# AI-ON/Few-Shot-Music-Generation

Measured on AMD Instinct MI355X. Metric: episodes/s (LSTM-baseline train step, synthetic vocab=10k seq_len=128 5-way/5-shot h=512), higher is better.
Workload: dtype f32 (bf16x3-split products, fp32 accumulate)

## Files before the change

few-shot-music-generation_amd/csrc/api_debug.hip:

```cpp
#include "fsmg_model.h"

using namespace fsmg;
using namespace fsmg_host;


extern "C" {

int fsmg_debug_clock_begin(fsmg_handle h, int32_t microseconds) {
    if (!h || microseconds <= 0 || microseconds > 1000000) return FSMG_ERR_INVALID;
    BEGIN_CALL(h, true);
    if (!h->probe) HIPCK(h, hipStreamCreateWithFlags(&h->probe, hipStreamNonBlocking));
    if (!h->d_probe) HIPCK(h, hipMalloc((void**)&h->d_probe, 64));
    HIPCK(h, hipMemsetAsync(h->d_probe, 0, 64, h->probe));
    HIPCK(h, launch_clock_probe(h->probe, (long long)microseconds * 100, h->d_probe));
    return FSMG_OK;
}
int fsmg_debug_clock_end(fsmg_handle h, float* ghz) {
    if (!h || !ghz) return FSMG_ERR_INVALID;
    if (!h->probe || !h->d_probe) return fail(h, FSMG_ERR_STATE, "fsmg_debug_clock_end without fsmg_debug_clock_begin");
    BEGIN_CALL(h, true);
    unsigned long long v[2] = {0, 0};
    HIPCK(h, hipStreamSynchronize(h->probe));
    HIPCK(h, hipMemcpy(v, h->d_probe, sizeof(v), hipMemcpyDeviceToHost));
    *ghz = v[1] ? (float)((double)v[0] / (double)v[1] * 0.1) : 0.0f;
    return FSMG_OK;
}

int fsmg_debug_dims(fsmg_handle h, int32_t dims[5]) {
    if (!h || !dims) return FSMG_ERR_INVALID;
    dims[0] = h->Ep; dims[1] = h->Hp; dims[2] = h->V1p; dims[3] = h->lastB; dims[4] = h->T;
    return FSMG_OK;
}

int fsmg_debug_read(fsmg_handle h, const char* what, float* host, int64_t count) {
    if (!h || !what || !host || count <= 0) return FSMG_ERR_INVALID;
    BEGIN_CALL(h);
    const int64_t B = h->lastB, T = h->T, Hp = h->Hp, G4 = h->G4, rows = T * B;
    const float* src = nullptr; int64_t cap = 0;
    auto layer_of = [&](const char* prefix) -> int {
        const size_t n = std::strlen(prefix);
        if (std::strncmp(what, prefix, n) != 0) return -1;
        const int l = std::atoi(what + n);
        return (l >= 0 && l < h->L && std::strlen(what) > n) ? l : -1;
    };
    int l;
    if (!std::strcmp(what, "aux_tries")) { host[0] = (float)h->aux_tries; return FSMG_OK; }
    if (!std::strcmp(what, "fused_softmax")) { host[0] = h->fused_softmax ? 1.0f : 0.0f; if (count > 1) host[1] = h->fs_call ? 1.0f : 0.0f; return FSMG_OK; }
    if (!std::strcmp(what, "xcd_bx3")) { host[0] = h->xcd_bx3 ? 1.0f : 0.0f; return FSMG_OK; }
    if (!std::strcmp(what, "gemm_kinds")) {
        for (int64_t i = 0; i < count && i < 4; ++i) host[i] = (float)h->gemm_kinds[i];
        return FSMG_OK;
    }
    if (!std::strcmp(what, "xov_selfcheck")) {
        const float v[3] = {(float)h->xov_selfcheck_runs, (float)h->xov_passes, (float)h->xov_selfcheck_every};
        for (int64_t i = 0; i < count && i < 3; ++i) host[i] = v[i];
        return FSMG_OK;
    }
    if (!std::strcmp(what, "xcd_partitioned")) {
        host[0] = h->xov ? 1.0f : 0.0f;
        if (count > 1) { const int b = h->lastB > 0 ? h->lastB : 45, rpx = lstm_xcd16_packed_rows(b, h->Hp); host[1] = (h->xov && rpx > 0) ? (float)xov_first_free(b, h->Hp) : 8.0f; }
        if (count > 2) host[2] = h->xov_last ? 1.0f : 0.0f;
        return FSMG_OK;
    }
    if (!std::strcmp(what, "logits")) { src = h->logits; cap = rows * h->V1p; }
    else if (!std::strcmp(what, "dlogits")) { src = dlogits_buf(h); cap = rows * h->V1p; }
    else if (!std::strcmp(what, "lse")) { src = h->lse; cap = rows; }
    else if (!std::strcmp(what, "ce")) { src = h->ce; cap = rows; }
    else if (!std::strcmp(what, "dx")) { src = h->dXemb; cap = rows * h->Ep; }
    else if (!std::strcmp(what, "dh")) { src = h->dH; cap = rows * Hp; }
    else if (!std::strcmp(what, "gnorm")) { src = h->d_gnorm; cap = 1; }
    else if (!std::strcmp(what, "tail")) { src = h->G + h->n_flat; cap = FSMG_GRAD_TAIL; }
    else if ((l = layer_of("gates")) >= 0) { src = h->Z[l]; cap = rows * G4; }
    else if ((l = layer_of("h")) >= 0) { src = h->Hs[l]; cap = (T + 1) * B * Hp; }
    else if ((l = layer_of("c")) >= 0) { src = h->Cs[l]; cap = (T + 1) * B * Hp; }
    else return fail(h, FSMG_ERR_NAME, std::string("unknown debug buffer '") + what + "'");
    if (count > cap) return fail(h, FSMG_ERR_SIZE, "debug read larger than the buffer");
    HIPCK(h, hipStreamSynchronize(h->stream));
    HIPCK(h, hipMemcpy(host, src, sizeof(float) * count, hipMemcpyDeviceToHost));
    return FSMG_OK;
}

int fsmg_debug_step_profile(fsmg_handle h, int32_t which, uint64_t* stamps, int64_t cap, int32_t* n_blocks,
                            int32_t* n_waves) {
    if (!h || !stamps || !n_blocks || !n_waves || h->lastB <= 0 || h->T < 3) return FSMG_ERR_INVALID;
    BEGIN_CALL(h);
    { const int rc_cs = ensure_cs(h); if (rc_cs != FSMG_OK) return rc_cs; }
    const int B = h->lastB, Hp = h->Hp, G4 = h->G4, l = h->L - 1, t = h->T / 2;
    const int nb = which == 0 ? (G4 / 16) * ((B + 15) / 16) : (Hp / 16) * ((B + 15) / 16);
    const int nw = which == 0 ? 4 : 8;
    const int64_t n = (int64_t)nb * nw * 8;
    if (cap < n) return fail(h, FSMG_ERR_SIZE, "stamp buffer too small");
    unsigned long long* d = nullptr;
    HIPCK(h, hipMalloc((void**)&d, sizeof(unsigned long long) * n));
    HIPCK(h, hipMemsetAsync(d, 0, sizeof(unsigned long long) * n, h->stream));
    for (int rep = 0; rep < 3; ++rep) {
        if (which == 0) {
            LstmFwdArgs a{};
            const size_t Bp16 = (size_t)(B + 15) / 16 * 16;
            a.KhF = h->khf + (size_t)(2 * l) * Hp * G4; a.hF_prev = h->HF[l] + (size_t)t * Bp16 * Hp;
            a.hF_next = h->HF[l] + (size_t)(t + 1) * Bp16 * Hp; a.z = h->Z[l] + (size_t)t * B * G4;
            a.c_prev = h->Cs[l] + (size_t)t * B * Hp; a.c_next = h->Cs[l] + (size_t)(t + 1) * B * Hp;
            a.h_next = h->Hs[l] + (size_t)(t + 1) * B * Hp; a.B = B; a.Hp = Hp;
            HIPCK(h, launch_lstm_fwd_step(h->stream, a, d));
        } else {
            LstmBwdArgs a{};
            const size_t Bp16 = (size_t)(B + 15) / 16 * 16;
            a.KhF = h->khf + (size_t)(2 * l + 1) * Hp * G4; a.dzF_next = h->dzF + (size_t)((t + 1) & 1) * Bp16 * G4;
            a.dzF_cur = h->dzF + (size_t)(t & 1) * Bp16 * G4; a.gates = h->Z[l] + (size_t)t * B * G4;
            a.c_t = h->Cs[l] + (size_t)(t + 1) * B * Hp; a.c_prev = h->Cs[l] + (size_t)t * B * Hp; a.dc = h->dC;
            a.dh_top = h->dH + (size_t)t * B * Hp; a.B = B; a.Hp = Hp;
            HIPCK(h, launch_lstm_bwd_step(h->stream, a, d));
        }
    }
    HIPCK(h, hipStreamSynchronize(h->stream));
    HIPCK(h, hipMemcpy(stamps, d, sizeof(unsigned long long) * n, hipMemcpyDeviceToHost));
    hipFree(d);
    *n_blocks = nb; *n_waves = nw;
    return FSMG_OK;
}

int fsmg_timing_enable(fsmg_handle h, int32_t on) {
    if (!h) return FSMG_ERR_INVALID;
    BEGIN_CALL(h);
    drain_timers(h);
    h->timing = on != 0;
    return FSMG_OK;
}
int fsmg_timing_select(fsmg_handle h, const char* kernel_class) {
    if (!h) return FSMG_ERR_INVALID;
    BEGIN_CALL(h);
    drain_timers(h);
    h->timing_only = kernel_class ? kernel_class : "";
    return FSMG_OK;
}
int fsmg_timing_read(fsmg_handle h, const char* kernel_class, double* total_ms, int64_t* launches) {
    if (!h || !kernel_class) return FSMG_ERR_INVALID;
    BEGIN_CALL(h);
    drain_timers(h);
    auto it = h->timers.find(kernel_class);
    if (total_ms) *total_ms = it == h->timers.end() ? 0.0 : it->second.total_ms;
    if (launches) *launches = it == h->timers.end() ? 0 : it->second.launches;
    return FSMG_OK;
}
int fsmg_timing_reset(fsmg_handle h) {
    if (!h) return FSMG_ERR_INVALID;
    BEGIN_CALL(h);
    drain_timers(h);
    h->timers.clear();
    return FSMG_OK;
}

}
```

few-shot-music-generation_amd/csrc/elementwise.hip:

```cpp
#include <algorithm>
#include "fsmg_kernels.h"
#include <cstdlib>

namespace fsmg {
namespace {

__device__ __forceinline__ float wave_sum(float v) {
#pragma unroll
    for (int o = 32; o > 0; o >>= 1) v += __shfl_xor(v, o, 64);
    return v;
}
__device__ __forceinline__ double wave_sum_d(double v) {
#pragma unroll
    for (int o = 32; o > 0; o >>= 1) v += __shfl_xor(v, o, 64);
    return v;
}
__device__ __forceinline__ float wave_max(float v) {
#pragma unroll
    for (int o = 32; o > 0; o >>= 1) v = fmaxf(v, __shfl_xor(v, o, 64));
    return v;
}

__global__ __launch_bounds__(256) void k_fill32(uint32_t* __restrict__ p, uint32_t word, long long n) {
    const long long n4 = n >> 2;
    const uint4 w4 = make_uint4(word, word, word, word);
    for (long long i = (long long)blockIdx.x * 256 + threadIdx.x; i < n4; i += (long long)gridDim.x * 256)
        reinterpret_cast<uint4*>(p)[i] = w4;
    if (blockIdx.x == 0 && threadIdx.x < (n & 3)) p[(n4 << 2) + threadIdx.x] = word;
}

__global__ __launch_bounds__(256) void k_fill32_if(const int* __restrict__ cond, uint32_t* __restrict__ p, uint32_t word, long long n) {
    if (*cond == 0) return;
    const long long n4 = n >> 2;
    const uint4 w4 = make_uint4(word, word, word, word);
    for (long long i = (long long)blockIdx.x * 256 + threadIdx.x; i < n4; i += (long long)gridDim.x * 256)
        reinterpret_cast<uint4*>(p)[i] = w4;
    if (blockIdx.x == 0 && threadIdx.x < (n & 3)) p[(n4 << 2) + threadIdx.x] = word;
}

constexpr int SQ_CHUNK = 256 * 16;
__global__ __launch_bounds__(256) void k_multi_op(const MultiOps r) {
    const MultiOp& o = r.op[blockIdx.y];
    if (o.kind == MULTI_FILL) {
        if (o.cond != nullptr && *o.cond == 0) return;
        uint32_t* p = (uint32_t*)o.dst;
        const uint32_t word = o.word;
        const long long n = o.n, n4 = n >> 2;
        const uint4 w4 = make_uint4(word, word, word, word);
        for (long long i = (long long)blockIdx.x * 256 + threadIdx.x; i < n4; i += (long long)gridDim.x * 256)
            reinterpret_cast<uint4*>(p)[i] = w4;
        if (blockIdx.x == 0 && threadIdx.x < (n & 3)) p[(n4 << 2) + threadIdx.x] = word;
        return;
    }
    __shared__ double sh[4];
    if (o.kind == MULTI_MEAN) {
        if (blockIdx.x != 0) return;
        const int tid = threadIdx.x, lane = tid & 63, wave = tid >> 6;
        const float* x = (const float*)o.src;
        const int n = (int)o.n;
        double l = 0.0;
        for (int i0 = tid; i0 < n; i0 += 256 * 16) {
            float b[16];
#pragma unroll
            for (int k = 0; k < 16; ++k) b[k] = (i0 + 256 * k < n) ? x[i0 + 256 * k] : 0.0f;
#pragma unroll
            for (int k = 0; k < 16; ++k) if (i0 + 256 * k < n) l += (double)b[k];
        }
        l = wave_sum_d(l);
        if (lane == 0) sh[wave] = l;
        __syncthreads();
        if (tid == 0) *(float*)o.dst = (float)(((sh[0] + sh[1]) + (sh[2] + sh[3])) / ((double)n + 1e-12));
        return;
    }
    const int tid = threadIdx.x, lane = tid & 63, wave = tid >> 6;
    const float* sl = (const float*)o.src;
    float* out = (float*)o.dst;
    const long long n = o.n, nchunks = (n + SQ_CHUNK - 1) / SQ_CHUNK;
    const bool vec = (o.stride & 3) == 0 && (n & 3) == 0;
    if (o.sq == nullptr && vec) {
        const long long n4 = n >> 2;
        for (long long i = (long long)blockIdx.x * 256 + tid; i < n4; i += (long long)gridDim.x * 256) {
            float4 v = *reinterpret_cast<const float4*>(sl + 4 * i);
            int z = 1;
            for (; z + 3 < o.nslab; z += 4) {
                const float4 w0 = *reinterpret_cast<const float4*>(sl + z * o.stride + 4 * i);
                const float4 w1 = *reinterpret_cast<const float4*>(sl + (z + 1) * o.stride + 4 * i);
                const float4 w2 = *reinterpret_cast<const float4*>(sl + (z + 2) * o.stride + 4 * i);
                const float4 w3 = *reinterpret_cast<const float4*>(sl + (z + 3) * o.stride + 4 * i);
                v.x += w0.x; v.y += w0.y; v.z += w0.z; v.w += w0.w;
                v.x += w1.x; v.y += w1.y; v.z += w1.z; v.w += w1.w;
                v.x += w2.x; v.y += w2.y; v.z += w2.z; v.w += w2.w;
                v.x += w3.x; v.y += w3.y; v.z += w3.z; v.w += w3.w;
            }
            for (; z < o.nslab; ++z) {
                const float4 w = *reinterpret_cast<const float4*>(sl + z * o.stride + 4 * i);
                v.x += w.x; v.y += w.y; v.z += w.z; v.w += w.w;
            }
            if (o.row_scale != nullptr) {
                const float c = o.row_scale[(4 * i) / o.row_len];
                v.x *= c; v.y *= c; v.z *= c; v.w *= c;
            }
            *reinterpret_cast<float4*>(out + 4 * i) = v;
        }
        return;
    }
    for (long long c = blockIdx.x; c < nchunks; c += gridDim.x) {
        const long long base = c * SQ_CHUNK;
        double s = 0.0;
        if (vec && base + SQ_CHUNK <= n) {
            float4 v[4];
#pragma unroll
            for (int i = 0; i < 4; ++i) v[i] = *reinterpret_cast<const float4*>(sl + base + 4 * (tid + 256 * i));
            int z = 1;
            for (; z + 1 < o.nslab; z += 2) {
                float4 w0[4], w1[4];
#pragma unroll
                for (int i = 0; i < 4; ++i) {
                    w0[i] = *reinterpret_cast<const float4*>(sl + z * o.stride + base + 4 * (tid + 256 * i));
                    w1[i] = *reinterpret_cast<const float4*>(sl + (z + 1) * o.stride + base + 4 * (tid + 256 * i));
                }
#pragma unroll
                for (int i = 0; i < 4; ++i) {
                    v[i].x += w0[i].x; v[i].y += w0[i].y; v[i].z += w0[i].z; v[i].w += w0[i].w;
                    v[i].x += w1[i].x; v[i].y += w1[i].y; v[i].z += w1[i].z; v[i].w += w1[i].w;
                }
            }
            if (z < o.nslab) {
#pragma unroll
                for (int i = 0; i < 4; ++i) {
                    const float4 w = *reinterpret_cast<const float4*>(sl + z * o.stride + base + 4 * (tid + 256 * i));
                    v[i].x += w.x; v[i].y += w.y; v[i].z += w.z; v[i].w += w.w;
                }
            }
#pragma unroll
            for (int i = 0; i < 4; ++i) {
                *reinterpret_cast<float4*>(out + base + 4 * (tid + 256 * i)) = v[i];
                s += ((double)v[i].x * v[i].x + (double)v[i].y * v[i].y) + ((double)v[i].z * v[i].z + (double)v[i].w * v[i].w);
            }
        } else {
#pragma unroll
            for (int i = 0; i < 4; ++i) {
                const long long idx = base + 4 * (tid + 256 * i);
                float q[4] = {0.f, 0.f, 0.f, 0.f};
                int k = 0;
                for (long long j = idx; j < n && j < idx + 4; ++j, ++k) {
                    float v = sl[j];
                    for (int z = 1; z < o.nslab; ++z) v += sl[z * o.stride + j];
                    out[j] = v;
                    q[k] = v;
                }
                if (k == 4) s += ((double)q[0] * q[0] + (double)q[1] * q[1]) + ((double)q[2] * q[2] + (double)q[3] * q[3]);
                else for (int e = 0; e < k; ++e) s += (double)q[e] * q[e];
            }
        }
        if (o.sq != nullptr) {
            s = wave_sum_d(s);
            if (lane == 0) sh[wave] = s;
            __syncthreads();
            if (tid == 0) o.sq[c] = (sh[0] + sh[1]) + (sh[2] + sh[3]);
            __syncthreads();
        }
    }
}

__global__ void k_token_prep(const int* __restrict__ support, int n_support, const int* __restrict__ query,
                             int n_query, int T, int vocab, int start_word, int* __restrict__ X,
                             int* __restrict__ Y, int* __restrict__ err_flag, int* __restrict__ tok_first, int* __restrict__ tok_count) {
    __shared__ int s_key[512], s_cnt[512], s_min[512];
    const int B = n_support + n_query;
    const long long total = (long long)B * T;
    for (long long i0 = (long long)blockIdx.x * blockDim.x; i0 < total; i0 += (long long)gridDim.x * blockDim.x) {
        const long long i = i0 + threadIdx.x;
        const bool valid = i < total;
        const int b = valid ? (int)(i / T) : 0, t = valid ? (int)(i % T) : 0;
        int tok = 0;
        if (valid) {
            const int* row = (b < n_support) ? support + (long long)b * T : query + (long long)(b - n_support) * T;
            tok = row[t];
            if (tok < 0 || tok >= vocab) {
                atomicOr(err_flag, 1);
                tok = min(max(tok, 0), vocab - 1);
            }
            Y[(long long)t * B + b] = tok;
            if (t + 1 < T) X[(long long)(t + 1) * B + b] = tok;
            if (t == 0) X[b] = start_word;
        }
        if (tok_first != nullptr) {
            for (int j = threadIdx.x; j < 512; j += blockDim.x) { s_key[j] = -1; s_cnt[j] = 0; s_min[j] = 0x7FFFFFFF; }
            __syncthreads();
            if (valid && t + 1 < T) {
                const int pos = (int)((long long)(t + 1) * B + b);
                unsigned slot = ((unsigned)tok * 2654435761u) >> 23;
                bool placed = false;
#pragma unroll 1
                for (int probe = 0; probe < 8 && !placed; ++probe) {
                    const int prev = atomicCAS(&s_key[slot], -1, tok);
                    if (prev == -1 || prev == tok) { atomicAdd(&s_cnt[slot], 1); atomicMin(&s_min[slot], pos); placed = true; }
                    else slot = (slot + 1) & 511u;
                }
                if (!placed) { atomicMin(tok_first + tok, pos); atomicAdd(tok_count + tok, 1); }
            }
            __syncthreads();
            for (int j = threadIdx.x; j < 512; j += blockDim.x)
                if (s_key[j] >= 0) { atomicMin(tok_first + s_key[j], s_min[j]); atomicAdd(tok_count + s_key[j], s_cnt[j]); }
            __syncthreads();
            if (valid && t == 0) { atomicMin(tok_first + start_word, b); atomicAdd(tok_count + start_word, 1); }
        }
    }
}

__global__ void k_gather_rows(const int* __restrict__ table, const int* __restrict__ idx, int n_rows, int T, int n_songs,
                              int* __restrict__ out, int* __restrict__ err_flag) {
    const long long total = (long long)n_rows * T;
    for (long long i = (long long)blockIdx.x * blockDim.x + threadIdx.x; i < total; i += (long long)gridDim.x * blockDim.x) {
        const int r = (int)(i / T), t = (int)(i % T);
        int song = idx[r];
        if (song < 0 || song >= n_songs) { atomicOr(err_flag, 1); song = 0; }
        out[i] = table[(long long)song * T + t];
    }
}

__global__ __launch_bounds__(256) void k_ce_rows(const float* logits, int ld, int n_vocab,
                                                 const int* __restrict__ tgt, float* __restrict__ lse,
                                                 float* __restrict__ ce, float* dlogits, float inv_n) {
    __shared__ float sh[4];
    __shared__ float s_lse;
    const int r = blockIdx.x, tid = threadIdx.x, lane = tid & 63, wave = tid >> 6;
    const float* row = logits + (long long)r * ld;
    const int nv4 = n_vocab & ~3;
    float m = -INFINITY;
    for (int v = 4 * tid; v < nv4; v += 1024) {
        const float4 x = *reinterpret_cast<const float4*>(row + v);
        m = fmaxf(fmaxf(m, fmaxf(x.x, x.y)), fmaxf(x.z, x.w));
    }
    if (tid < n_vocab - nv4) m = fmaxf(m, row[nv4 + tid]);
    m = wave_max(m);
    if (lane == 0) sh[wave] = m;
    __syncthreads();
    m = fmaxf(fmaxf(sh[0], sh[1]), fmaxf(sh[2], sh[3]));
    __syncthreads();
    float s = 0.0f;
    for (int v = 4 * tid; v < nv4; v += 1024) {
        const float4 x = *reinterpret_cast<const float4*>(row + v);
        s += (expf(x.x - m) + expf(x.y - m)) + (expf(x.z - m) + expf(x.w - m));
    }
    if (tid < n_vocab - nv4) s += expf(row[nv4 + tid] - m);
    s = wave_sum(s);
    if (lane == 0) sh[wave] = s;
    __syncthreads();
    const int t = tgt[r];
    if (tid == 0) {
        const float l = m + logf((sh[0] + sh[1]) + (sh[2] + sh[3]));
        lse[r] = l;
        ce[r] = l - row[t];
        s_lse = l;
    }
    if (dlogits == nullptr) return;
    __syncthreads();
    const float l = s_lse;
    float* drow = dlogits + (long long)r * ld;
    for (int v = 4 * tid; v < ld; v += 1024) {
        const float4 x = *reinterpret_cast<const float4*>(row + v);
        float4 d;
        d.x = (v + 0 < n_vocab) ? (expf(x.x - l) - (v + 0 == t ? 1.0f : 0.0f)) * inv_n : 0.0f;
        d.y = (v + 1 < n_vocab) ? (expf(x.y - l) - (v + 1 == t ? 1.0f : 0.0f)) * inv_n : 0.0f;
        d.z = (v + 2 < n_vocab) ? (expf(x.z - l) - (v + 2 == t ? 1.0f : 0.0f)) * inv_n : 0.0f;
        d.w = (v + 3 < n_vocab) ? (expf(x.w - l) - (v + 3 == t ? 1.0f : 0.0f)) * inv_n : 0.0f;
        __builtin_nontemporal_store(d.x, drow + v); __builtin_nontemporal_store(d.y, drow + v + 1);
        __builtin_nontemporal_store(d.z, drow + v + 2); __builtin_nontemporal_store(d.w, drow + v + 3);
    }
}

template <int NV, bool NT>
__device__ __forceinline__ void ce_row_reg(float* sh, const int r, const float* logits, int ld, int n_vocab, const int* __restrict__ tgt,
                                           float* __restrict__ lse, float* __restrict__ ce, float* dlogits, float inv_n) {
    const int tid = threadIdx.x, lane = tid & 63, wave = tid >> 6;
    const float* row = logits + (long long)r * ld;
    float4 x[NV];
    float m = -INFINITY;
#pragma unroll
    for (int i = 0; i < NV; ++i) {
        const int v = 4 * tid + 1024 * i;
        x[i] = make_float4(-INFINITY, -INFINITY, -INFINITY, -INFINITY);
        if (v < ld) {
            const float4 q = *reinterpret_cast<const float4*>(row + v);
            x[i].x = (v + 0 < n_vocab) ? q.x : -INFINITY; x[i].y = (v + 1 < n_vocab) ? q.y : -INFINITY;
            x[i].z = (v + 2 < n_vocab) ? q.z : -INFINITY; x[i].w = (v + 3 < n_vocab) ? q.w : -INFINITY;
        }
        m = fmaxf(fmaxf(m, fmaxf(x[i].x, x[i].y)), fmaxf(x[i].z, x[i].w));
    }
    m = wave_max(m);
    if (lane == 0) sh[wave] = m;
    __syncthreads();
    m = fmaxf(fmaxf(sh[0], sh[1]), fmaxf(sh[2], sh[3]));
    const int t = tgt[r];
    float s = 0.0f, xt = 0.0f;
#pragma unroll
    for (int i = 0; i < NV; ++i) {
        const int v = 4 * tid + 1024 * i;
        if (t >= v && t < v + 4) xt = (t == v) ? x[i].x : (t == v + 1) ? x[i].y : (t == v + 2) ? x[i].z : x[i].w;
        x[i].x = expf(x[i].x - m); x[i].y = expf(x[i].y - m); x[i].z = expf(x[i].z - m); x[i].w = expf(x[i].w - m);
        s += (x[i].x + x[i].y) + (x[i].z + x[i].w);
    }
    s = wave_sum(s);
    xt = wave_sum(xt);
    if (lane == 0) { sh[4 + wave] = s; }
    __syncthreads();
    s = (sh[4] + sh[5]) + (sh[6] + sh[7]);
    const int tw = ((t >> 2) & 255) >> 6;
    if (wave == tw && lane == 0) {
        const float l = m + logf(s);
        lse[r] = l;
        ce[r] = l - xt;
    }
    if (dlogits == nullptr) return;
    const float scale = inv_n / s;
    float* drow = dlogits + (long long)r * ld;
#pragma unroll
    for (int i = 0; i < NV; ++i) {
        const int v = 4 * tid + 1024 * i;
        if (v < ld) {
            float4 d;
            d.x = x[i].x * scale - (v + 0 == t ? inv_n : 0.0f);
            d.y = x[i].y * scale - (v + 1 == t ? inv_n : 0.0f);
            d.z = x[i].z * scale - (v + 2 == t ? inv_n : 0.0f);
            d.w = x[i].w * scale - (v + 3 == t ? inv_n : 0.0f);
            if (NT) {
                __builtin_nontemporal_store(d.x, drow + v); __builtin_nontemporal_store(d.y, drow + v + 1);
                __builtin_nontemporal_store(d.z, drow + v + 2); __builtin_nontemporal_store(d.w, drow + v + 3);
            } else {
                *reinterpret_cast<float4*>(drow + v) = d;
            }
        }
    }
}

template <int NV, bool NT>
__global__ __launch_bounds__(256) void k_ce_rows_reg(const float* logits, int ld, int n_vocab,
                                                     const int* __restrict__ tgt, float* __restrict__ lse,
                                                     float* __restrict__ ce, float* dlogits, float inv_n) {
    __shared__ float sh[8];
    ce_row_reg<NV, NT>(sh, blockIdx.x, logits, ld, n_vocab, tgt, lse, ce, dlogits, inv_n);
}

__global__ __launch_bounds__(256) void k_ce_combine(const float2* __restrict__ part, int nparts,
                                                    const float* __restrict__ tgt_logit, int rows, float* __restrict__ ce) {
    const int lane = threadIdx.x & 63, row = blockIdx.x * 4 + (threadIdx.x >> 6);
    if (row >= rows) return;
    const float2* p = part + (long long)row * nparts;
    float m = -INFINITY;
    for (int i = lane; i < nparts; i += 64) m = fmaxf(m, p[i].x);
    m = wave_max(m);
    float s = 0.0f;
    for (int i = lane; i < nparts; i += 64) {
        const float2 v = p[i];
        if (v.x > -INFINITY) s += v.y * expf(v.x - m);
    }
    s = wave_sum(s);
    if (lane == 0) ce[row] = m + logf(s) - tgt_logit[row];
}

__global__ __launch_bounds__(256) void k_ce_finish(const float2* __restrict__ part, int nparts,
                                                   const int* __restrict__ tgt, int rows, float inv_n, float* E, int ld,
                                                   float* __restrict__ lse, float* __restrict__ ce, float* __restrict__ crow,
                                                   const float* __restrict__ hs, float* __restrict__ hs_scaled, int hp,
                                                   int* err_flag, unsigned long long* range_counter) {
    const int lane = threadIdx.x & 63, row = blockIdx.x * 4 + (threadIdx.x >> 6);
    if (blockIdx.x == 0 && threadIdx.x < 32) crow[rows + threadIdx.x] = 0.0f;
    if (row >= rows) return;
    const float2* p = part + (long long)row * nparts;
    float S = 0.0f;
    for (int i = lane; i < nparts; i += 64) S += p[i].y;
    S = wave_sum(S);
    const float c = inv_n / S;
    if (lane == 0) {
        float* e = E + (long long)row * ld + tgt[row];
        const float et = *e;
        const float l = logf(S);
        lse[row] = l;
        ce[row] = l - logf(et);
        crow[row] = c;
        if (!(S >= CE_SUM_MIN && S <= CE_SUM_MAX && et >= CE_TGT_MIN)) {
            atomicCAS(err_flag, 0, 4);
            crow[row] = 0.0f;
            atomicAdd_system(range_counter, 1ull);
            __threadfence_system();
        } else {
            *e = et - S;
        }
    }
    const float* hrow = hs + (long long)row * hp;
    float* orow = hs_scaled + (long long)row * hp;
    for (int i = 4 * lane; i < hp; i += 256) {
        float4 v = *reinterpret_cast<const float4*>(hrow + i);
        v.x *= c; v.y *= c; v.z *= c; v.w *= c;
        *reinterpret_cast<float4*>(orow + i) = v;
    }
}

__global__ __launch_bounds__(256) void k_scale_rows(float* C, const float* __restrict__ row_scale, long long n4, int n_per_row4) {
    for (long long i = (long long)blockIdx.x * 256 + threadIdx.x; i < n4; i += (long long)gridDim.x * 256) {
        const float c = row_scale[i / n_per_row4];
        float4 v = reinterpret_cast<float4*>(C)[i];
        v.x *= c; v.y *= c; v.z *= c; v.w *= c;
        reinterpret_cast<float4*>(C)[i] = v;
    }
}

__global__ __launch_bounds__(256) void k_loss_reduce(const float* __restrict__ ce, int T, int B, int rpg,
                                                     float* __restrict__ out) {
    __shared__ double sh[4];
    const int g = blockIdx.x, tid = threadIdx.x, lane = tid & 63, wave = tid >> 6;
    const int n = T * rpg;
    double s = 0.0;
    for (int i = tid; i < n; i += 256) {
        const int t = i / rpg, b = g * rpg + i % rpg;
        s += (double)ce[(long long)t * B + b];
    }
    s = wave_sum_d(s);
    if (lane == 0) sh[wave] = s;
    __syncthreads();
    if (tid == 0) out[g] = (float)(((sh[0] + sh[1]) + (sh[2] + sh[3])) / ((double)n + 1e-12));
}

__device__ __forceinline__ void sum_partials_body(const double* __restrict__ partials, int n, float* dst,
                                                  const int* flag_src, const float* __restrict__ ce, int ce_n, float* loss_out) {
    __shared__ double sh[4];
    const int tid = threadIdx.x, lane = tid & 63, wave = tid >> 6;
    double s = 0.0;
    for (int i = tid; i < n; i += 256) s += partials[i];
    s = wave_sum_d(s);
    if (lane == 0) sh[wave] = s;
    __syncthreads();
    if (tid == 0) {
        dst[0] = (float)((sh[0] + sh[1]) + (sh[2] + sh[3]));
        if (flag_src != nullptr) {
            dst[2] = (*flag_src == 2) ? 1.0f : 0.0f; dst[3] = (*flag_src == 1) ? 1.0f : 0.0f; dst[4] = 0.0f;
            dst[5] = (*flag_src == 4) ? 1.0f : 0.0f;
        }
    }
    if (ce == nullptr) return;
    __syncthreads();
    double l = 0.0;
    for (int i0 = tid; i0 < ce_n; i0 += 256 * 16) {
        float b[16];
#pragma unroll
        for (int k = 0; k < 16; ++k) b[k] = (i0 + 256 * k < ce_n) ? ce[i0 + 256 * k] : 0.0f;
#pragma unroll
        for (int k = 0; k < 16; ++k) if (i0 + 256 * k < ce_n) l += (double)b[k];
    }
    l = wave_sum_d(l);
    if (lane == 0) sh[wave] = l;
    __syncthreads();
    if (tid == 0) *loss_out = (float)(((sh[0] + sh[1]) + (sh[2] + sh[3])) / ((double)ce_n + 1e-12));
}


constexpr int EMBED_HEAVY = 48;
__global__ __launch_bounds__(256) void k_embed_grad_chunks(const int* __restrict__ X, int n, const float* __restrict__ dX, int Ep,
                                                           float* __restrict__ part, const int* __restrict__ tok_count, const SumPartialsArgs sp) {
    if (blockIdx.x == (unsigned)((n + 255) / 256)) { sum_partials_body(sp.partials, sp.n, sp.dst, sp.flag_src, sp.ce, sp.ce_n, sp.loss_out); return; }
    __shared__ unsigned long long mask[4];
    __shared__ __attribute__((aligned(16))) float wsum[4][1024];
    const int base = blockIdx.x * 256, tid = threadIdx.x, lane = tid & 63, wave = tid >> 6, i = base + tid;
    const int tok = (i < n) ? X[i] : -1;
    bool pending = (i < n) && tok_count[tok] > EMBED_HEAVY;
    for (;;) {
        const unsigned long long pb = __ballot(pending);
        if (lane == 0) mask[wave] = pb;
        __syncthreads();
        int first = -1;
#pragma unroll
        for (int w = 0; w < 4; ++w) if (first < 0 && mask[w]) first = 64 * w + __ffsll((long long)mask[w]) - 1;
        __syncthreads();
        if (first < 0) break;
        const int tk = X[base + first];
        const bool hit = pending && tok == tk;
        const unsigned long long hb = __ballot(hit);
        if (lane == 0) mask[wave] = hb;
        __syncthreads();
        {
            float4 a4[4];
#pragma unroll
            for (int c = 0; c < 4; ++c) a4[c] = make_float4(0.f, 0.f, 0.f, 0.f);
            unsigned long long mk = mask[wave];
            const int nf4 = Ep >> 2;
            while (mk) {
                int bits[4];
#pragma unroll
                for (int k = 0; k < 4; ++k) { bits[k] = mk ? __ffsll((long long)mk) - 1 : -1; mk &= mk - 1; }
                float4 v[4][4];
#pragma unroll
                for (int k = 0; k < 4; ++k) {
                    const float4* src = reinterpret_cast<const float4*>(dX + (long long)(base + 64 * wave + max(bits[k], 0)) * Ep);
#pragma unroll
                    for (int c = 0; c < 4; ++c) v[k][c] = (bits[k] >= 0 && lane + 64 * c < nf4) ? src[lane + 64 * c] : make_float4(0.f, 0.f, 0.f, 0.f);
                }
#pragma unroll
                for (int k = 0; k < 4; ++k)
                    if (bits[k] >= 0) {
#pragma unroll
                        for (int c = 0; c < 4; ++c) { a4[c].x += v[k][c].x; a4[c].y += v[k][c].y; a4[c].z += v[k][c].z; a4[c].w += v[k][c].w; }
                    }
            }
#pragma unroll
            for (int c = 0; c < 4; ++c)
                if (lane + 64 * c < nf4) reinterpret_cast<float4*>(&wsum[wave][0])[lane + 64 * c] = a4[c];
        }
        __syncthreads();
#pragma unroll
        for (int c = 0; c < 4; ++c)
            if (tid + 256 * c < Ep) {
                const int col = tid + 256 * c;
                part[(long long)(base + first) * Ep + col] = ((wsum[0][col] + wsum[1][col]) + wsum[2][col]) + wsum[3][col];
            }
        if (hit) pending = false;
        __syncthreads();
    }
}

__global__ __launch_bounds__(256) void k_embed_grad(const int* __restrict__ X, int n, const float* __restrict__ dX,
                                                    int Ep, float* __restrict__ dEmb, int* __restrict__ tok_first, int* __restrict__ tok_count,
                                                    const float* __restrict__ part) {
    __shared__ unsigned long long mask[4];
    const int r = blockIdx.x, tid = threadIdx.x, lane = tid & 63, wave = tid >> 6;
    const int tok = X[r];
    int want = n + 1;
    if (tok_first != nullptr) {
        if (tok_first[tok] != r) return;
        want = tok_count[tok];
        if (part != nullptr && want > EMBED_HEAVY) {
            float acc[4] = {0.f, 0.f, 0.f, 0.f};
            int found = 0;
            for (int base = r & ~255; base < n && found < want; base += 256) {
                const int i = base + tid;
                const bool hit = (i < n) && (X[i] == tok);
                const unsigned long long bal = __ballot(hit);
                if (lane == 0) mask[wave] = bal;
                __syncthreads();
                int first = -1;
#pragma unroll
                for (int w = 0; w < 4; ++w) {
                    found += __popcll(mask[w]);
                    if (first < 0 && mask[w]) first = 64 * w + __ffsll((long long)mask[w]) - 1;
                }
                if (first >= 0) {
                    const float* src = part + (long long)(base + first) * Ep;
#pragma unroll
                    for (int c = 0; c < 4; ++c)
                        if (tid + 256 * c < Ep) acc[c] += src[tid + 256 * c];
                }
                __syncthreads();
            }
#pragma unroll
            for (int c = 0; c < 4; ++c)
                if (tid + 256 * c < Ep) dEmb[(long long)tok * Ep + tid + 256 * c] = acc[c];
            if (tid == 0) { tok_first[tok] = 0x7FFFFFFF; tok_count[tok] = 0; }
            return;
        }
    } else {
        int dup = 0;
        for (int i = tid; i < r; i += 256) dup |= (X[i] == tok);
        if (__syncthreads_or(dup)) return;
    }

    float acc[4] = {0.f, 0.f, 0.f, 0.f};
    int found = 0;
    for (int base = r; base < n && found < want; base += 256) {
        const int i = base + tid;
        const bool hit = (i < n) && (X[i] == tok);
        const unsigned long long bal = __ballot(hit);
        if (lane == 0) mask[wave] = bal;
        __syncthreads();
#pragma unroll
        for (int w = 0; w < 4; ++w) {
            unsigned long long mk = mask[w];
            found += __popcll(mk);
            while (mk) {
                const int bit = __ffsll((long long)mk) - 1;
                mk &= mk - 1;
                const float* src = dX + (long long)(base + 64 * w + bit) * Ep;
#pragma unroll
                for (int c = 0; c < 4; ++c)
                    if (tid + 256 * c < Ep) acc[c] += src[tid + 256 * c];
            }
        }
        __syncthreads();
    }
#pragma unroll
    for (int c = 0; c < 4; ++c)
        if (tid + 256 * c < Ep) dEmb[(long long)tok * Ep + tid + 256 * c] = acc[c];
    if (tok_first != nullptr && tid == 0) { tok_first[tok] = 0x7FFFFFFF; tok_count[tok] = 0; }
}

__global__ __launch_bounds__(256) void k_sqnorm_partials(const float* __restrict__ x, long long n,
                                                         double* __restrict__ partials) {
    __shared__ double sh[4];
    const int tid = threadIdx.x, lane = tid & 63, wave = tid >> 6;
    const long long base = (long long)blockIdx.x * SQ_CHUNK;
    double s = 0.0;
#pragma unroll
    for (int i = 0; i < 4; ++i) {
        const long long idx = base + 4 * (tid + 256 * i);
        if (idx + 3 < n) {
            const float4 v = *reinterpret_cast<const float4*>(x + idx);
            s += ((double)v.x * v.x + (double)v.y * v.y) + ((double)v.z * v.z + (double)v.w * v.w);
        } else {
            for (long long j = idx; j < n && j < idx + 4; ++j) s += (double)x[j] * x[j];
        }
    }
    s = wave_sum_d(s);
    if (lane == 0) sh[wave] = s;
    __syncthreads();
    if (tid == 0) partials[blockIdx.x] = (sh[0] + sh[1]) + (sh[2] + sh[3]);
}

__global__ __launch_bounds__(256) void k_adam_update(const UpdateArgs a) {
    __shared__ double sh[4];
    __shared__ float s_scale, s_alpha;
    const int tid = threadIdx.x, lane = tid & 63, wave = tid >> 6;
    if (a.consume != nullptr) {
        if (a.consume[0] == 0.0f) return;
        if (tid == 0) { s_scale = a.consume[1]; s_alpha = a.consume[2]; }
    } else {
    if ((a.err_flag != nullptr && *a.err_flag != 0) || a.tail[2] != 0.0f || a.tail[3] != 0.0f || a.tail[4] != 0.0f || a.tail[5] != 0.0f) {
        if (a.publish != nullptr && blockIdx.x == 0 && tid == 0) a.publish[0] = 0.0f;
        return;
    }
    double s = 0.0;
    for (int i = tid; i < a.n_partials; i += 256) s += a.partials[i];
    s = wave_sum_d(s);
    if (lane == 0) sh[wave] = s;
    __syncthreads();
    if (tid == 0) {
        double sq = ((sh[0] + sh[1]) + (sh[2] + sh[3])) * (double)a.grad_scale * (double)a.grad_scale;
        if (a.use_slices) sq += (double)a.tail[0] * (double)a.grad_scale * (double)a.grad_scale;
        const double gnorm = sqrt(sq);
        const double clip = (double)a.clip;
        s_scale = (float)(clip / fmax(gnorm, clip) * (double)a.grad_scale);
        const long long step = *a.step;
        const double t = (double)(step + 1);
        const double lr_s = (double)a.lr * pow(0.5, (double)step / (double)a.n_decay);
        s_alpha = (float)(lr_s * sqrt(1.0 - pow(0.999, t)) / (1.0 - pow(0.9, t)));
        if (a.gnorm_out != nullptr && blockIdx.x == 0) *a.gnorm_out = (float)gnorm;
        if (a.publish != nullptr && blockIdx.x == 0) { a.publish[0] = 1.0f; a.publish[1] = s_scale; a.publish[2] = s_alpha; }
    }
    }
    __syncthreads();
    const float scale = s_scale, alpha = s_alpha;
    const float b1 = 0.9f, b2 = 0.999f, eps = 1e-8f;
    const long long n4 = a.n >> 2;
    for (long long i = (long long)blockIdx.x * 256 + tid; i < n4; i += (long long)gridDim.x * 256) {
        float4 g = reinterpret_cast<const float4*>(a.g)[i];
        float4 m = reinterpret_cast<float4*>(a.m)[i];
        float4 v = reinterpret_cast<float4*>(a.v)[i];
        float4 p = reinterpret_cast<float4*>(a.p)[i];
#define FSMG_ADAM1(c)                                         \
        {                                                     \
            const float gc = g.c * scale;                     \
            m.c = b1 * m.c + (1.0f - b1) * gc;                \
            v.c = b2 * v.c + (1.0f - b2) * gc * gc;           \
            p.c = p.c - alpha * m.c / (sqrtf(v.c) + eps);     \
        }
        FSMG_ADAM1(x) FSMG_ADAM1(y) FSMG_ADAM1(z) FSMG_ADAM1(w)
#undef FSMG_ADAM1
        reinterpret_cast<float4*>(a.m)[i] = m;
        reinterpret_cast<float4*>(a.v)[i] = v;
        reinterpret_cast<float4*>(a.p)[i] = p;
    }
}

__global__ __launch_bounds__(256) void k_sgd_update(const UpdateArgs a) {
    __shared__ double sh[4];
    __shared__ float s_scale;
    if ((a.err_flag != nullptr && *a.err_flag != 0) || a.tail[2] != 0.0f || a.tail[3] != 0.0f || a.tail[4] != 0.0f || a.tail[5] != 0.0f) return;
    const int tid = threadIdx.x, lane = tid & 63, wave = tid >> 6;
    double s = 0.0;
    for (int i = tid; i < a.n_partials; i += 256) s += a.partials[i];
    s = wave_sum_d(s);
    if (lane == 0) sh[wave] = s;
    __syncthreads();
    if (tid == 0) {
        double sq = (sh[0] + sh[1]) + (sh[2] + sh[3]);
        if (a.use_slices) sq += (double)a.tail[0];
        const double gnorm = sqrt(sq), clip = (double)a.clip;
        s_scale = (float)(clip / fmax(gnorm, clip)) * a.lr;
        if (a.gnorm_out != nullptr && blockIdx.x == 0) *a.gnorm_out = (float)gnorm;
    }
    __syncthreads();
    const float step = s_scale;
    const long long n4 = a.n >> 2;
    for (long long i = (long long)blockIdx.x * 256 + tid; i < n4; i += (long long)gridDim.x * 256) {
        const float4 g = reinterpret_cast<const float4*>(a.g)[i];
        float4 p = reinterpret_cast<float4*>(a.p)[i];
        p.x -= step * g.x; p.y -= step * g.y; p.z -= step * g.z; p.w -= step * g.w;
        reinterpret_cast<float4*>(a.p)[i] = p;
    }
}

__global__ void k_step_increment(const StepIncArgs a) {
    if (threadIdx.x != 0 || blockIdx.x != 0) return;
    step_increment_body(a);
}

__global__ __launch_bounds__(256) void k_sum_partials(const double* __restrict__ partials, int n, float* dst,
                                                      const int* flag_src, const float* __restrict__ ce, int ce_n, float* loss_out) {
    sum_partials_body(partials, n, dst, flag_src, ce, ce_n, loss_out);
}

__global__ void k_clock_probe(long long ticks, unsigned long long* out) {
    const unsigned long long r0 = __builtin_amdgcn_s_memrealtime(), c0 = __builtin_amdgcn_s_memtime();
    unsigned long long r1 = r0;
    while ((long long)(r1 - r0) < ticks) { __builtin_amdgcn_s_sleep(64); r1 = __builtin_amdgcn_s_memrealtime(); }
    const unsigned long long c1 = __builtin_amdgcn_s_memtime();
    if (threadIdx.x == 0) { out[0] = c1 - c0; out[1] = r1 - r0; }
}

__global__ __launch_bounds__(256) void k_copy_words(uint4* __restrict__ dst, const uint4* __restrict__ src, long long n4) {
    for (long long i = (long long)blockIdx.x * 256 + threadIdx.x; i < n4; i += (long long)gridDim.x * 256) dst[i] = src[i];
}

__global__ __launch_bounds__(256) void k_compare_words(const uint4* __restrict__ a, const uint4* __restrict__ b, long long n4, int* err_flag,
                                                       unsigned long long* counter) {
    if (*err_flag != 0) return;
    unsigned bad = 0;
    for (long long i = (long long)blockIdx.x * 256 + threadIdx.x; i < n4; i += (long long)gridDim.x * 256) {
        const uint4 x = a[i], y = b[i];
        bad += (x.x != y.x) | (x.y != y.y) | (x.z != y.z) | (x.w != y.w);
    }
    const unsigned long long votes = __ballot(bad != 0);
    if (votes == 0) return;
    unsigned total = bad;
    for (int o = 32; o > 0; o >>= 1) total += __shfl_xor(total, o);
    if ((threadIdx.x & 63) == __ffsll((long long)votes) - 1) {
        atomicAdd_system(counter, (unsigned long long)total);
        *err_flag = 2;
        __threadfence_system();
    }
}

__global__ void k_queue_probe(int* flag, int* out, int role, long long ticks) {
    if (threadIdx.x != 0) return;
    if (role == 1) { __hip_atomic_store(flag, 1, __ATOMIC_RELAXED, __HIP_MEMORY_SCOPE_AGENT); return; }
    const unsigned long long t0 = __builtin_amdgcn_s_memrealtime();
    int seen = 0;
    while ((long long)(__builtin_amdgcn_s_memrealtime() - t0) < ticks) {
        if (__hip_atomic_load(flag, __ATOMIC_RELAXED, __HIP_MEMORY_SCOPE_AGENT) != 0) { seen = 1; break; }
        __builtin_amdgcn_s_sleep(16);
    }
    out[0] = seen;
}

__global__ void k_unigram_update(const int* __restrict__ words, long long n, unsigned* __restrict__ counts, int vocab, int* err_flag) {
    for (long long i = (long long)blockIdx.x * blockDim.x + threadIdx.x; i < n; i += (long long)gridDim.x * blockDim.x) {
        const int w = words[i];
        if (w < 0 || w >= vocab) { atomicOr(err_flag, 1); continue; }
        atomicAdd(counts + w, 1u);
    }
}
__global__ __launch_bounds__(1024) void k_unigram_nll(const int* __restrict__ words, long long n, const unsigned* __restrict__ counts, int vocab,
                                                      float* out, int* err_flag) {
    __shared__ double sh[16];
    __shared__ float s_total;
    const int tid = threadIdx.x, lane = tid & 63, wave = tid >> 6;
    double s = 0.0;
    for (int i = tid; i < vocab; i += 1024) s += (double)counts[i];
    s = wave_sum_d(s);
    if (lane == 0) sh[wave] = s;
    __syncthreads();
    if (tid == 0) { double t = 0.0; for (int w = 0; w < 16; ++w) t += sh[w]; s_total = (float)t; }
    __syncthreads();
    const float total = s_total;
    double l = 0.0;
    for (long long i = tid; i < n; i += 1024) {
        const int w = words[i];
        if (w < 0 || w >= vocab) { atomicOr(err_flag, 1); continue; }
        l += (double)logf((float)counts[w] / total);
    }
    l = wave_sum_d(l);
    __syncthreads();
    if (lane == 0) sh[wave] = l;
    __syncthreads();
    if (tid == 0) { double t = 0.0; for (int w = 0; w < 16; ++w) t += sh[w]; out[0] = (float)(-t / (double)(n > 0 ? n : 1)); out[1] = total; }
}
__global__ __launch_bounds__(1024) void k_unigram_argmax(const unsigned* __restrict__ counts, int vocab, int* out) {
    __shared__ unsigned sc[1024];
    __shared__ int si[1024];
    const int tid = threadIdx.x;
    unsigned best = 0; int bi = 0x7FFFFFFF;
    for (int i = tid; i < vocab; i += 1024) { const unsigned c = counts[i]; if (c > best || (c == best && i < bi)) { best = c; bi = i; } }
    sc[tid] = best; si[tid] = bi;
    __syncthreads();
    for (int o = 512; o > 0; o >>= 1) {
        if (tid < o) {
            const unsigned c = sc[tid + o]; const int i = si[tid + o];
            if (c > sc[tid] || (c == sc[tid] && i < si[tid])) { sc[tid] = c; si[tid] = i; }
        }
        __syncthreads();
    }
    if (tid == 0) *out = si[0];
}

}

hipError_t launch_token_prep(hipStream_t s, const int* support, int n_support, const int* query, int n_query,
                             int T, int vocab, int start_word, int* X, int* Y, int* err_flag, int* tok_first, int* tok_count) {
    const long long total = (long long)(n_support + n_query) * T;
    if (total <= 0) return hipSuccess;
    int blocks = (int)((total + 255) / 256);
    if (blocks > 1024) blocks = 1024;
    hipLaunchKernelGGL(k_token_prep, dim3(blocks), dim3(256), 0, s, support, n_support, query, n_query, T, vocab,
                       start_word, X, Y, err_flag, tok_first, tok_count);
    return hipGetLastError();
}

hipError_t launch_ce_rows(hipStream_t s, const float* logits, int ld, int rows, int n_vocab, const int* tgt,
                          float* lse, float* ce, float* dlogits, float inv_n) {
    if (rows <= 0) return hipSuccess;
    static const int nt = std::getenv("FSMG_CE_NT") ? (std::atoi(std::getenv("FSMG_CE_NT")) != 0) : 1;
    if (ld <= 6 * 1024) {
        if (nt) hipLaunchKernelGGL((k_ce_rows_reg<6, true>), dim3(rows), dim3(256), 0, s, logits, ld, n_vocab, tgt, lse, ce, dlogits, inv_n);
        else hipLaunchKernelGGL((k_ce_rows_reg<6, false>), dim3(rows), dim3(256), 0, s, logits, ld, n_vocab, tgt, lse, ce, dlogits, inv_n);
    } else if (ld <= 12 * 1024) {
        if (nt) hipLaunchKernelGGL((k_ce_rows_reg<12, true>), dim3(rows), dim3(256), 0, s, logits, ld, n_vocab, tgt, lse, ce, dlogits, inv_n);
        else hipLaunchKernelGGL((k_ce_rows_reg<12, false>), dim3(rows), dim3(256), 0, s, logits, ld, n_vocab, tgt, lse, ce, dlogits, inv_n);
    }
    else hipLaunchKernelGGL(k_ce_rows, dim3(rows), dim3(256), 0, s, logits, ld, n_vocab, tgt, lse, ce, dlogits, inv_n);
    return hipGetLastError();
}

hipError_t launch_ce_combine(hipStream_t s, const float2* part, int nparts, const float* tgt_logit, int rows, float* ce) {
    if (rows <= 0) return hipSuccess;
    hipLaunchKernelGGL(k_ce_combine, dim3((rows + 3) / 4), dim3(256), 0, s, part, nparts, tgt_logit, rows, ce);
    return hipGetLastError();
}

hipError_t launch_ce_finish(hipStream_t s, const float2* part, int nparts, const int* tgt, int rows, float inv_n,
                            float* E, int ld, float* lse, float* ce, float* crow, const float* hs, float* hs_scaled, int hp,
                            int* err_flag, long long* range_counter) {
    if (rows <= 0) return hipSuccess;
    if ((hp & 3) != 0 || err_flag == nullptr || range_counter == nullptr) return hipErrorInvalidValue;
    hipLaunchKernelGGL(k_ce_finish, dim3((rows + 3) / 4), dim3(256), 0, s, part, nparts, tgt, rows, inv_n, E, ld, lse, ce, crow,
                       hs, hs_scaled, hp, err_flag, (unsigned long long*)range_counter);
    return hipGetLastError();
}

hipError_t launch_scale_rows(hipStream_t s, float* C, const float* row_scale, int M, int N) {
    if (M <= 0 || N <= 0) return hipSuccess;
    if ((N & 3) != 0) return hipErrorInvalidValue;
    const long long n4 = (long long)M * N / 4;
    hipLaunchKernelGGL(k_scale_rows, dim3((int)std::min<long long>((n4 + 255) / 256, 2048)), dim3(256), 0, s, C, row_scale, n4, N / 4);
    return hipGetLastError();
}

hipError_t launch_loss_reduce(hipStream_t s, const float* ce, int T, int B, int rows_per_group, int ngroups,
                              float* out) {
    hipLaunchKernelGGL(k_loss_reduce, dim3(ngroups), dim3(256), 0, s, ce, T, B, rows_per_group, out);
    return hipGetLastError();
}

hipError_t launch_embed_grad(hipStream_t s, const int* X, int n, const float* dX, int Ep, float* dEmb, int* tok_first, int* tok_count, float* part,
                             const SumPartialsArgs* sum) {
    if (n <= 0) return sum != nullptr ? hipErrorInvalidValue : hipSuccess;
    if (Ep > 1024) return hipErrorInvalidValue;
    if (tok_first == nullptr || tok_count == nullptr || (Ep & 3) != 0 || ((uintptr_t)dX & 15) != 0) part = nullptr;
    if (part == nullptr && sum != nullptr) return hipErrorInvalidValue;
    if (part != nullptr) {
        SumPartialsArgs sp{};
        if (sum != nullptr) sp = *sum;
        hipLaunchKernelGGL(k_embed_grad_chunks, dim3((n + 255) / 256 + (sum != nullptr ? 1 : 0)), dim3(256), 0, s, X, n, dX, Ep, part, tok_count, sp);
    }
    hipLaunchKernelGGL(k_embed_grad, dim3(n), dim3(256), 0, s, X, n, dX, Ep, dEmb, tok_first, tok_count, part);
    return hipGetLastError();
}

hipError_t launch_multi_op(hipStream_t s, const MultiOps& r) {
    if (r.count <= 0) return hipSuccess;
    long long bx = 1;
    for (int k = 0; k < r.count; ++k) {
        const long long want = r.op[k].kind == MULTI_FILL ? (r.op[k].n / 4 + 255) / 256 : r.op[k].kind == MULTI_MEAN ? 1 :
                               (r.op[k].sq == nullptr ? (r.op[k].n / 4 + 255) / 256 : (r.op[k].n + SQ_CHUNK - 1) / SQ_CHUNK);
        bx = std::max(bx, want);
    }
    bx = std::max<long long>(1, std::min<long long>(bx, 1024));
    hipLaunchKernelGGL(k_multi_op, dim3((int)bx, r.count), dim3(256), 0, s, r);
    return hipGetLastError();
}

hipError_t launch_gather_rows(hipStream_t s, const int* table, const int* idx, int n_rows, int T, int n_songs, int* out, int* err_flag) {
    if (n_rows <= 0) return hipSuccess;
    const long long total = (long long)n_rows * T;
    hipLaunchKernelGGL(k_gather_rows, dim3((int)std::min<long long>((total + 255) / 256, 1024)), dim3(256), 0, s, table, idx, n_rows, T, n_songs, out, err_flag);
    return hipGetLastError();
}

hipError_t launch_fill32_if(hipStream_t s, const int* cond, void* p, uint32_t word, long long n_words) {
    if (n_words <= 0) return hipSuccess;
    long long blocks = (n_words / 4 + 255) / 256;
    if (blocks > 2048) blocks = 2048;
    if (blocks < 1) blocks = 1;
    hipLaunchKernelGGL(k_fill32_if, dim3((int)blocks), dim3(256), 0, s, cond, (uint32_t*)p, word, n_words);
    return hipGetLastError();
}

hipError_t launch_fill32(hipStream_t s, void* p, uint32_t word, long long n_words) {
    if (n_words <= 0) return hipSuccess;
    long long blocks = (n_words / 4 + 255) / 256;
    if (blocks > 2048) blocks = 2048;
    if (blocks < 1) blocks = 1;
    hipLaunchKernelGGL(k_fill32, dim3((int)blocks), dim3(256), 0, s, (uint32_t*)p, word, n_words);
    return hipGetLastError();
}

int sqnorm_blocks(long long n) { return (int)((n + SQ_CHUNK - 1) / SQ_CHUNK); }

hipError_t launch_sqnorm_partials(hipStream_t s, const float* x, long long n, double* partials) {
    const int nb = sqnorm_blocks(n);
    if (nb <= 0) return hipSuccess;
    hipLaunchKernelGGL(k_sqnorm_partials, dim3(nb), dim3(256), 0, s, x, n, partials);
    return hipGetLastError();
}

hipError_t launch_adam_update(hipStream_t s, const UpdateArgs& a) {
    long long n4 = a.n >> 2;
    int blocks = (int)((n4 + 255) / 256);
    if (blocks > 2048) blocks = 2048;
    if (blocks < 1) blocks = 1;
    hipLaunchKernelGGL(k_adam_update, dim3(blocks), dim3(256), 0, s, a);
    return hipGetLastError();
}

hipError_t launch_sgd_update(hipStream_t s, const UpdateArgs& a) {
    long long n4 = a.n >> 2;
    int blocks = (int)((n4 + 255) / 256);
    if (blocks > 2048) blocks = 2048;
    if (blocks < 1) blocks = 1;
    hipLaunchKernelGGL(k_sgd_update, dim3(blocks), dim3(256), 0, s, a);
    return hipGetLastError();
}

hipError_t launch_step_increment(hipStream_t s, const StepIncArgs& a) {
    hipLaunchKernelGGL(k_step_increment, dim3(1), dim3(64), 0, s, a);
    return hipGetLastError();
}

hipError_t launch_sum_partials(hipStream_t s, const double* partials, int n, float* dst, const int* flag_src,
                               const float* ce, int ce_n, float* loss_out) {
    hipLaunchKernelGGL(k_sum_partials, dim3(1), dim3(256), 0, s, partials, n, dst, flag_src, ce, ce_n, loss_out);
    return hipGetLastError();
}

hipError_t launch_queue_probe(hipStream_t s, int* flag, int* out, int role, long long realtime_ticks) {
    hipLaunchKernelGGL(k_queue_probe, dim3(1), dim3(64), 0, s, flag, out, role, realtime_ticks);
    return hipGetLastError();
}
hipError_t launch_clock_probe(hipStream_t s, long long realtime_ticks, unsigned long long* out) {
    hipLaunchKernelGGL(k_clock_probe, dim3(1), dim3(64), 0, s, realtime_ticks, out);
    return hipGetLastError();
}
hipError_t launch_copy_words(hipStream_t s, void* dst, const void* src, long long n_words) {
    const long long n4 = n_words >> 2;
    if (n4 <= 0) return hipSuccess;
    hipLaunchKernelGGL(k_copy_words, dim3((int)std::min<long long>((n4 + 255) / 256, 4096)), dim3(256), 0, s, (uint4*)dst, (const uint4*)src, n4);
    return hipGetLastError();
}
hipError_t launch_compare_words(hipStream_t s, const void* a, const void* b, long long n_words, int* err_flag, long long* counter) {
    const long long n4 = n_words >> 2;
    if (n4 <= 0) return hipSuccess;
    const int blocks = (int)std::min<long long>((n4 + 255) / 256, 4096);
    hipLaunchKernelGGL(k_compare_words, dim3(blocks), dim3(256), 0, s, (const uint4*)a, (const uint4*)b, n4, err_flag, (unsigned long long*)counter);
    return hipGetLastError();
}
hipError_t launch_unigram_update(hipStream_t s, const int* words, long long n, unsigned* counts, int vocab, int* err_flag) {
    if (n <= 0) return hipSuccess;
    hipLaunchKernelGGL(k_unigram_update, dim3((int)std::min<long long>((n + 255) / 256, 1024)), dim3(256), 0, s, words, n, counts, vocab, err_flag);
    return hipGetLastError();
}
hipError_t launch_unigram_nll(hipStream_t s, const int* words, long long n, const unsigned* counts, int vocab, float* out, int* err_flag) {
    hipLaunchKernelGGL(k_unigram_nll, dim3(1), dim3(1024), 0, s, words, n, counts, vocab, out, err_flag);
    return hipGetLastError();
}
hipError_t launch_unigram_argmax(hipStream_t s, const unsigned* counts, int vocab, int* out) {
    hipLaunchKernelGGL(k_unigram_argmax, dim3(1), dim3(1024), 0, s, counts, vocab, out);
    return hipGetLastError();
}

}
```

Baseline: 638.8.

## Rewrite embedding gradient as one-wave-per-row kernel with batched row gathers

Replaces the block-per-row embedding gradient kernel, on the path that has occurrence tables, with a wave-per-row kernel. Four rows go to each 256-thread block, and each row's own dX is loaded before the early-exit check. The owning wave scans 1024 tokens per iteration using ballots, collects the positions that match into a lane-distributed list, and then gathers and sums those rows in batches with float4 loads. This removes the __syncthreads and the shared-mask round trips, and cuts the number of launched blocks by four. The cost is extra register pressure, and each token's scan now runs in a single wave rather than a whole block.

```diff
diff --git a/few-shot-music-generation_amd/csrc/api_debug.hip b/few-shot-music-generation_amd/csrc/api_debug.hip
--- a/few-shot-music-generation_amd/csrc/api_debug.hip
+++ b/few-shot-music-generation_amd/csrc/api_debug.hip
@@ -60,6 +60,16 @@
         host[0] = h->xov ? 1.0f : 0.0f;
         if (count > 1) { const int b = h->lastB > 0 ? h->lastB : 45, rpx = lstm_xcd16_packed_rows(b, h->Hp); host[1] = (h->xov && rpx > 0) ? (float)xov_first_free(b, h->Hp) : 8.0f; }
         if (count > 2) host[2] = h->xov_last ? 1.0f : 0.0f;
+        return FSMG_OK;
+    }
+    if (!std::strcmp(what, "tok_first") || !std::strcmp(what, "tok_count")) {
+        const int* tab = what[4] == 'f' ? h->tok_first : h->tok_count;
+        if (tab == nullptr) return fail(h, FSMG_ERR_STATE, "this handle has no occurrence table");
+        if (count > h->V1) return fail(h, FSMG_ERR_SIZE, "debug read larger than the buffer");
+        std::vector<int> tmp((size_t)count);
+        HIPCK(h, hipStreamSynchronize(h->stream));
+        HIPCK(h, hipMemcpy(tmp.data(), tab, sizeof(int) * count, hipMemcpyDeviceToHost));
+        for (int64_t i = 0; i < count; ++i) host[i] = (float)tmp[i];
         return FSMG_OK;
     }
     if (!std::strcmp(what, "logits")) { src = h->logits; cap = rows * h->V1p; }
diff --git a/few-shot-music-generation_amd/csrc/elementwise.hip b/few-shot-music-generation_amd/csrc/elementwise.hip
--- a/few-shot-music-generation_amd/csrc/elementwise.hip
+++ b/few-shot-music-generation_amd/csrc/elementwise.hip
@@ -519,9 +519,88 @@
     }
 }
 
+template <int NC>
+__global__ __launch_bounds__(256) void k_embed_grad_wave(const int* __restrict__ X, int n, const float* __restrict__ dX, int Ep,
+                                                         float* __restrict__ dEmb, int* __restrict__ tok_first, int* __restrict__ tok_count,
+                                                         const float* __restrict__ part) {
+    const int lane = threadIdx.x & 63, p = blockIdx.x * 4 + __builtin_amdgcn_readfirstlane(threadIdx.x >> 6);
+    if (p >= n) return;
+    const int nf4 = Ep >> 2;
+    float4 own[NC];
+#pragma unroll
+    for (int c = 0; c < NC; ++c) own[c] = reinterpret_cast<const float4*>(dX + (long long)p * Ep)[min(lane + 64 * c, nf4 - 1)];
+    const int tok = __builtin_amdgcn_readfirstlane(X[p]);
+    const int first = __builtin_amdgcn_readfirstlane(tok_first[tok]), want = __builtin_amdgcn_readfirstlane(tok_count[tok]);
+#pragma unroll
+    for (int c = 0; c < NC; ++c) asm volatile("" : "+v"(own[c].x), "+v"(own[c].y), "+v"(own[c].z), "+v"(own[c].w));
+    if (first != p) return;
+    const bool heavy = want > EMBED_HEAVY;
+    const float* const src = heavy ? part : dX;
+    float4 a4[NC];
+#pragma unroll
+    for (int c = 0; c < NC; ++c) a4[c] = make_float4(0.f, 0.f, 0.f, 0.f);
+    int mine = 0, nlist = 0;
+    constexpr int R = 16 / NC;
+    auto add_listed = [&]() {
+        for (int j = 0; j < nlist; j += R) {
+            int pos[R];
+            float4 v[R][NC];
+#pragma unroll
+            for (int k = 0; k < R; ++k) {
+                pos[k] = (j + k < nlist) ? __shfl(mine, j + k, 64) : -1;
+                const float4* row = reinterpret_cast<const float4*>(src + (long long)max(pos[k], 0) * Ep);
+#pragma unroll
+                for (int c = 0; c < NC; ++c) v[k][c] = (pos[k] >= 0 && lane + 64 * c < nf4) ? row[lane + 64 * c] : make_float4(0.f, 0.f, 0.f, 0.f);
+            }
+#pragma unroll
+            for (int k = 0; k < R; ++k)
+                if (pos[k] >= 0) {
+#pragma unroll
+                    for (int c = 0; c < NC; ++c) { a4[c].x += v[k][c].x; a4[c].y += v[k][c].y; a4[c].z += v[k][c].z; a4[c].w += v[k][c].w; }
+                }
+        }
+        nlist = 0;
+    };
+    auto list = [&](int pos) {
+        if (lane == nlist) mine = pos;
+        ++nlist;
+    };
+    int found = 0, listed_chunk = -1;
+    if (!heavy) {
+#pragma unroll
+        for (int c = 0; c < NC; ++c) { a4[c].x += own[c].x; a4[c].y += own[c].y; a4[c].z += own[c].z; a4[c].w += own[c].w; }
+        found = 1;
+    }
+    for (int base = heavy ? (p & ~255) : p + 1; base < n && found < want; base += 1024) {
+        int x[16];
+#pragma unroll
+        for (int g = 0; g < 16; ++g) x[g] = (base + 64 * g + lane < n) ? X[base + 64 * g + lane] : -1;
+        bool any = false;
+#pragma unroll
+        for (int g = 0; g < 16; ++g) any |= x[g] == tok;
+        if (__ballot(any) == 0) continue;
+        if (nlist > 60) add_listed();
+#pragma unroll
+        for (int g = 0; g < 16; ++g) {
+            unsigned long long bal = __ballot(x[g] == tok);
+            found += __popcll(bal);
+            if (!heavy) {
+                while (bal) { list(base + 64 * g + __ffsll((long long)bal) - 1); bal &= bal - 1; }
+            } else {
+                const int chunk = (base + 64 * g) >> 8;
+                if (bal && chunk != listed_chunk) { list(base + 64 * g + __ffsll((long long)bal) - 1); listed_chunk = chunk; }
+            }
+        }
+    }
+    add_listed();
+#pragma unroll
+    for (int c = 0; c < NC; ++c)
+        if (lane + 64 * c < nf4) reinterpret_cast<float4*>(dEmb + (long long)tok * Ep)[lane + 64 * c] = a4[c];
+    if (lane == 0) { tok_first[tok] = 0x7FFFFFFF; tok_count[tok] = 0; }
+}
+
 __global__ __launch_bounds__(256) void k_embed_grad(const int* __restrict__ X, int n, const float* __restrict__ dX,
-                                                    int Ep, float* __restrict__ dEmb, int* __restrict__ tok_first, int* __restrict__ tok_count,
-                                                    const float* __restrict__ part) {
+                                                    int Ep, float* __restrict__ dEmb, int* __restrict__ tok_first, int* __restrict__ tok_count) {
     __shared__ unsigned long long mask[4];
     const int r = blockIdx.x, tid = threadIdx.x, lane = tid & 63, wave = tid >> 6;
     const int tok = X[r];
@@ -529,35 +608,6 @@
     if (tok_first != nullptr) {
         if (tok_first[tok] != r) return;
         want = tok_count[tok];
-        if (part != nullptr && want > EMBED_HEAVY) {
-            float acc[4] = {0.f, 0.f, 0.f, 0.f};
-            int found = 0;
-            for (int base = r & ~255; base < n && found < want; base += 256) {
-                const int i = base + tid;
-                const bool hit = (i < n) && (X[i] == tok);
-                const unsigned long long bal = __ballot(hit);
-                if (lane == 0) mask[wave] = bal;
-                __syncthreads();
-                int first = -1;
-#pragma unroll
-                for (int w = 0; w < 4; ++w) {
-                    found += __popcll(mask[w]);
-                    if (first < 0 && mask[w]) first = 64 * w + __ffsll((long long)mask[w]) - 1;
-                }
-                if (first >= 0) {
-                    const float* src = part + (long long)(base + first) * Ep;
-#pragma unroll
-                    for (int c = 0; c < 4; ++c)
-                        if (tid + 256 * c < Ep) acc[c] += src[tid + 256 * c];
-                }
-                __syncthreads();
-            }
-#pragma unroll
-            for (int c = 0; c < 4; ++c)
-                if (tid + 256 * c < Ep) dEmb[(long long)tok * Ep + tid + 256 * c] = acc[c];
-            if (tid == 0) { tok_first[tok] = 0x7FFFFFFF; tok_count[tok] = 0; }
-            return;
-        }
     } else {
         int dup = 0;
         for (int i = tid; i < r; i += 256) dup |= (X[i] == tok);
@@ -870,7 +920,15 @@
         if (sum != nullptr) sp = *sum;
         hipLaunchKernelGGL(k_embed_grad_chunks, dim3((n + 255) / 256 + (sum != nullptr ? 1 : 0)), dim3(256), 0, s, X, n, dX, Ep, part, tok_count, sp);
     }
-    hipLaunchKernelGGL(k_embed_grad, dim3(n), dim3(256), 0, s, X, n, dX, Ep, dEmb, tok_first, tok_count, part);
+    if (part != nullptr) {
+        if (((uintptr_t)dEmb & 15) != 0) return hipErrorInvalidValue;
+        const dim3 grid((n + 3) / 4);
+        if (Ep <= 256) hipLaunchKernelGGL(k_embed_grad_wave<1>, grid, dim3(256), 0, s, X, n, dX, Ep, dEmb, tok_first, tok_count, part);
+        else if (Ep <= 512) hipLaunchKernelGGL(k_embed_grad_wave<2>, grid, dim3(256), 0, s, X, n, dX, Ep, dEmb, tok_first, tok_count, part);
+        else hipLaunchKernelGGL(k_embed_grad_wave<4>, grid, dim3(256), 0, s, X, n, dX, Ep, dEmb, tok_first, tok_count, part);
+    } else {
+        hipLaunchKernelGGL(k_embed_grad, dim3(n), dim3(256), 0, s, X, n, dX, Ep, dEmb, tok_first, tok_count);
+    }
     return hipGetLastError();
 }
 
```

After: 639.3 (median of 4 runs). About the same (+0.1%).
